# AmourWaltz/BayesLMs

Hardware: AMD Instinct MI355X
Metric: train_tokens_per_sec (higher is better)
Workload: dtype f32

## Files before the change

### bayeslms_amd/_lib.py

```python
import ctypes as C
import os

import torch

_HERE = os.path.dirname(os.path.abspath(__file__))
LIB_PATH = os.environ.get("BLM_LIB") or os.path.join(_HERE, "libbayeslm_hip.so")

ABI_VERSION = 1
TOPK_MAX = 256
OK = 0
ERR_INVALID, ERR_ABI, ERR_HIP, ERR_UNSUPPORTED = -1, -2, -3, -4
GEMM_NT, GEMM_NN, GEMM_TN = 0, 1, 2
EPI_NONE, EPI_BIAS, EPI_BIAS_GELU, EPI_MUL_DGELU, EPI_BAYES_WGRAD, EPI_GP_MIX, EPI_MUL_DGP_MIX = range(7)
GEMM_ACCUMULATE = 1
STREAM_WEIGHT = 0x10000000
STREAM_DROPOUT = 0x20000000
STREAM_LRT = 0x30000000

c_fp = C.POINTER(C.c_float)
c_i64p = C.POINTER(C.c_int64)


class Rng(C.Structure):
    _fields_ = [("seed", C.c_uint64), ("stream", C.c_uint32), ("step", C.c_uint32)]
# ... 32 lines not shown


class BeamPoolArgs(C.Structure):
    _fields_ = ([("abi_version", C.c_uint32), ("P", C.c_int32)]
                + [(n, C.c_void_p) for n in ("norm", "raw", "len", "step", "parent", "finished", "count", "inserted")])


class GemmPlan(C.Structure):
    _fields_ = [("tile", C.c_int32), ("splits", C.c_int32), ("source", C.c_int32), ("model_us", C.c_float)]


_vp, _i, _f, _i64 = C.c_void_p, C.c_int, C.c_float, C.c_int64
_rngp, _varp = C.POINTER(Rng), C.POINTER(Variational)
SIGNATURES = {
    "blm_abi_version": (C.c_uint32, []),
    "blm_last_error": (C.c_char_p, []),
    "blm_query": (_i, [_i, C.c_char_p, C.POINTER(_i), C.POINTER(_i)]),
    "blm_sample_weight": (_i, [_vp, _i64, _i64, _varp, _vp, _vp, _f, _vp]),
    "blm_sample_weight_bwd": (_i, [_vp, _i64, _i64, _varp, _vp, _vp, _vp]),
    "blm_variational_group_fwd": (_i, [C.POINTER(VarItem), _i, _vp, _vp]),
    "blm_variational_group_bwd": (_i, [C.POINTER(VarItem), _i, _vp, _vp]),
    "blm_philox_normal": (_i, [_vp, _i64, _rngp, _vp]),
    "blm_lrt_prepare": (_i, [_vp, _vp, _i64, _i, _vp]),
    "blm_lrt_combine": (_i, [_vp, _vp, _vp, _rngp, _i, _i, _i, _i, _i, _vp]),
    "blm_lrt_bwd_factor": (_i, [_vp, _vp, _vp, _vp, _rngp, _i, _i, _i, _i, _i, _vp]),
    "blm_lrt_mul": (_i, [_vp, _vp, _vp, _i64, _f, _i, _vp]),
    "blm_kl_mean_fwd": (_i, [_vp, _i64, _vp, _i64, _i64, _i, _f, _vp, _vp]),
    "blm_kl_mean_bwd": (_i, [_vp, _i64, _vp, _i64, _i64, _vp, _f, _vp, _i64, _vp, _vp]),
    "blm_gemm": (_i, [C.POINTER(GemmArgs), _vp]),
    "blm_set_gemm_mode": (_i, [_i]),
    "blm_get_gemm_mode": (_i, []),
    "blm_gemm_plan_query": (_i, [C.POINTER(GemmArgs), C.POINTER(GemmPlan)]),
    "blm_gemm_plan_launch": (_i, [C.POINTER(GemmArgs), C.POINTER(GemmPlan)]),
    "blm_gemm_plan_model_us": (_i, [C.POINTER(GemmArgs), _i, _i, C.POINTER(C.c_float)]),
    "blm_gemm_plan_override": (_i, [_i, _i]),
    "blm_gemm_plan_set": (_i, [_i] * 8),
    "blm_gemm_plan_clear": (_i, [_i]),
    "blm_mfma_probe_ws_floats": (_i64, []),
    "blm_mfma_probe": (_i, [_vp, _i, C.POINTER(C.c_double), _vp]),
    "blm_set_option": (_i, [C.c_char_p, _i]),
    "blm_get_option": (_i, [C.c_char_p, C.POINTER(C.c_int)]),
    "blm_gemm_plan_set_cus": (_i, [_i]),
    "blm_gemm_plan_get_cus": (_i, []),
    "blm_gemm_plan_comm_window": (_i, [_f]),
    "blm_gemm_plan_comm_window_left": (_f, []),
    "blm_gemm_plan_set_comm": (_i, [_i, _i, _i, _i, _i, _i, _i, _i]),
    "blm_embed_fwd": (_i, [_vp, _vp, _vp, _vp, _i, _i, _i, _i64, _f, _f, _rngp, _i, _i, _vp]),
    "blm_embed_bwd": (_i, [_vp, _vp, _vp, _i, _i, _i, _i64, _f, _f, _rngp, _i, _i, _vp]),
    "blm_add_pe_dropout": (_i, [_vp, _vp, _vp, _i, _i, _i, _f, _rngp, _i, _i, _vp]),
    "blm_dropout": (_i, [_vp, _vp, _i, _i, _i, _f, _rngp, _i, _i, _vp]),
    "blm_dropout_rows": (_i, [_vp, _vp, _i, _i, _i, _i, _f, _rngp, _i, _i, _vp]),
    "blm_add_dropout_ln_fwd": (_i, [_vp, _vp, _vp, _vp, _vp, _vp, _vp, _vp, _i, _i, _i, _f, _f, _rngp, _i, _i, _vp]),
    "blm_ln_bwd_ws_floats": (_i64, [_i, _i]),
    "blm_add_dropout_ln_bwd": (_i, [_vp, _vp, _vp, _vp, _vp, _vp, _vp, _vp, _vp, _vp, _i, _i, _i, _f, _rngp, _i, _i, _vp]),
    "blm_attn_fwd": (_i, [_vp, _vp, _vp, _i64, _vp, _vp, _i, _i, _i, _i, _f, _rngp, _i, _i, _vp]),
    "blm_attn_fwd_rows": (_i, [_vp, _vp, _vp, _i64, _vp, _vp, _i, _i, _i, _i, _vp]),
    "blm_attn_fwd_tree": (_i, [_vp, _vp, _vp, _i64, _vp, _vp, _vp, _i, _i, _i, _vp]),
    "blm_attn_bwd": (_i, [_vp, _vp, _vp, _i64, _vp, _vp, _vp, _vp, _vp, _vp, _i64, _i, _i, _i, _i, _f, _rngp, _i, _i, _vp]),
    "blm_attn_bwd_ws": (_i, [_vp, _vp, _vp, _i64, _vp, _vp, _vp, _vp, _vp, _vp, _i64, _i, _i, _i, _i, _f, _rngp, _i, _i, _vp,
                            _i64, _vp]),
    "blm_attn_bwd_ws_floats": (_i64, [_i, _i, _i, _i]),
    "blm_attn_fwd_keep": (_i, [_vp, _vp, _vp, _i64, _vp, _vp, _i, _i, _i, _i, _vp, _i, _i, _vp]),
    "blm_attn_bwd_keep": (_i, [_vp, _vp, _vp, _i64, _vp, _vp, _vp, _vp, _vp, _vp, _i64, _i, _i, _i, _i, _vp, _i, _i, _vp]),
    "blm_attn_decode_ws_floats": (_i64, [_i, _i, _i, _i, _i]),
    "blm_attn_decode": (_i, [_vp, _i64, _vp, _vp, _vp, _vp, _vp, _i64, _i, _i, _i, _i, _i, _i, _i, _vp]),
    "blm_kv_append": (_i, [_vp, _vp, _i64, _vp, _vp, _vp, _i, _i, _i, _i, _i, _i, _vp]),
    "blm_kv_gather": (_i, [_vp, _vp, _vp, _vp, _vp, _i, _i, _i, _i, _i, _i, _i, _vp]),
    "blm_embed_at": (_i, [_vp, _vp, _i64, _f, _vp, _vp, _i, _vp, _vp, _i, _i, _i, _vp]),
    "blm_log_softmax_rows": (_i, [_vp, _i64, _vp, _i64, _i, _i, _vp]),
    "blm_sample_rows": (_i, [_vp, _i64, _i, _i, _f, _rngp, _vp, _vp]),
    "blm_row_stats": (_i, [_vp, _i64, _vp, _i, _i, _vp, _vp, _vp, _vp, _vp, _vp]),
    "blm_topk_rows": (_i, [_vp, _i64, _i, _i, _i, _vp, _vp, _vp]),
    "blm_beam_select": (_i, [_vp, _vp, _vp, _vp, _i, _i, _i, _i64, _vp, _vp, _vp, _vp, _vp]),
    "blm_beam_select_pool": (_i, [_vp, _vp, _vp, _vp, _i, _i, _i, _i, _i64, _i, _i, _i, _f, _f, _i, C.POINTER(BeamPoolArgs),
                                  _vp, _vp, _vp, _vp, _vp, _vp, _vp]),
    "blm_sample_rows_filtered": (_i, [_vp, _i64, _i, _i, _f, _i, _f, _rngp, _vp, _vp]),
    "blm_ce_fwd_bwd": (_i, [_vp, _i64, _vp, _vp, _vp, _vp, _vp, _f, _i, _i, _vp]),
    "blm_ce_interp_fwd": (_i, [_vp, _vp, _i64, _f, _vp, _vp, _i, _i, _vp]),
    "blm_ce_soft_fwd_bwd": (_i, [_vp, _i64, _vp, _i64, _vp, _f, _vp, _vp, _vp, _vp, _vp, _vp, _vp, _f, _i, _i, _vp]),
    "blm_linear_nll_ws_floats": (_i64, [_i, _i]),
    "blm_linear_nll": (_i, [_vp, _i64, _vp, _i64, _vp, _vp, _vp, _vp, _vp, _i, _i, _i, _vp]),
    "blm_linear_mc_stats_ws_floats": (_i64, [_i, _i, _i]),
    "blm_linear_mc_stats": (_i, [_vp, _i64, _vp, _i64, _vp, _vp, _i, _vp, _vp, _vp, _vp, _vp, _i, _i, _i, _vp]),
    "blm_linear_mc_logprobs_ws_floats": (_i64, [_i, _i, _i]),
    "blm_linear_mc_logprobs": (_i, [_vp, _i64, _vp, _i64, _vp, _vp, _i, _vp, _i64, _vp, _vp, _vp, _vp, _vp, _i, _i, _i, _vp]),
    "blm_linear_nll2_wcat_floats": (_i64, [_i, _i, _i]),
    "blm_linear_nll2_ws_floats": (_i64, [_i, _i, _i, _i]),
    "blm_linear_nll2": (_i, [_vp, _i64, _vp, _i64, _vp, _i, _vp, _i64, _vp, _i64, _vp, _i, _f, _vp, _vp, _vp, _vp, _i, _vp, _i, _i, _vp]),
    "blm_linear_nll_edges_ws_floats": (_i64, [_i, _i]),
    "blm_linear_nll_edges": (_i, [_vp, _i64, _vp, _i64, _vp, _vp, _vp, _vp, _vp, _i, _i, _i, _i, _i, _vp]),
    "blm_linear_nll2_edges_ws_floats": (_i64, [_i, _i, _i, _i]),
    "blm_linear_nll2_edges": (_i, [_vp, _i64, _vp, _i64, _vp, _i, _vp, _i64, _vp, _i64, _vp, _i, _f, _vp, _vp, _vp, _vp, _i, _vp, _i, _i, _i,
                                   _vp]),
    "blm_ce_bwd": (_i, [_vp, _i64, _vp, _vp, _vp, _f, _vp, _i, _i, _vp]),
    "blm_gp_coef_grad": (_i, [_vp, _vp, _vp, _i, _i, _vp]),
    "blm_colsum": (_i, [_vp, _i64, _vp, _i, _i, _i, _vp]),
    "blm_colsum2": (_i, [_vp, _i64, _vp, _vp, _i, _i, _i, _vp]),
    "blm_init_multi": (_i, [_i, _vp, _vp, _vp, _vp, _vp]),
    "blm_sqnorm_ws_floats": (_i64, [_i]),
    "blm_sqnorm_multi": (_i, [_vp, _vp, _i, _vp, _vp, _vp]),
    "blm_clip_sgd_multi": (_i, [_vp, _vp, _vp, _vp, _i, _vp, _f, _f, _f, _i, _f, _vp]),
    "blm_lstm_step_fwd": (_i, [_vp, _vp, _vp, _vp, _vp, _vp, _vp, _vp, _i, _i, _vp]),
    "blm_lstm_step_bwd": (_i, [_vp] * 10 + [_i, _i, _vp]),
    "blm_lstm_seq_fwd": (_i, [_vp] * 6 + [_i, _i, _i, _vp]),
    "blm_lstm_seq_bwd": (_i, [_vp] * 7 + [_i, _vp, _i, _i, _i, _i, _i, _vp]),
    "blm_lstm_seq_pair_fwd": (_i, [_vp] * 5 + [_i] + [_vp] * 5 + [_i, _i, _i, _vp]),
# ... 172 lines not shown
```

### bayeslms_amd/csrc/elementwise.hip

```cpp
#include "blm_device.h"
#include "blm_host.h"
#include "blm_dropkey.h"

namespace blm {

constexpr int TPB = 256;

__global__ __launch_bounds__(TPB) void embed_fwd_kernel(const int64_t* __restrict__ ids, const float* __restrict__ enc,
                                                        const float* __restrict__ pe, float* __restrict__ out, int T,
                                                        int B, int D, long vocab, float scale, DropKey dk, bool vec) {
  const int lane = threadIdx.x & 63;
  const long row = (long)blockIdx.x * (TPB / 64) + (threadIdx.x >> 6);
  if (row >= (long)T * B) return;
  const int t = (int)(row / B), b = (int)(row % B);
  long id = ids[row];
  if (id < 0 || id >= vocab) id = 0;
  const float* e = enc + id * D;
  const float* pp = pe ? pe + (long)t * D : nullptr;
  float* o = out + row * D;
  if (vec) {
    for (int j = lane * 4; j < D; j += 256) {
      float4 v = *reinterpret_cast<const float4*>(e + j);
      float4 q = pp ? *reinterpret_cast<const float4*>(pp + j) : make_float4(0.f, 0.f, 0.f, 0.f);
      const float4 kp = keep4(dk, t, b, j);
// ... 140 lines not shown
    const float dx = s[v].x - mean, dy = s[v].y - mean, dz = s[v].z - mean, dw = s[v].w - mean;
    var += dx * dx + dy * dy + dz * dz + dw * dw;
  }
  const float rstd = rsqrtf(wave_sum(var) / D + eps);
  if (lane == 0) {
    if (mean_o) mean_o[row] = mean;
    if (rstd_o) rstd_o[row] = rstd;
  }
#pragma unroll
  for (int v = 0; v < VPT; ++v) {
    const int j = (v * 64 + lane) * 4;
    if (RAG && j >= D) continue;
    const float4 g = *reinterpret_cast<const float4*>(gamma + j);
    const float4 be = *reinterpret_cast<const float4*>(beta + j);
    if (s_out) *reinterpret_cast<float4*>(s_out + row * D + j) = s[v];
    float4 o;
    o.x = (s[v].x - mean) * rstd * g.x + be.x; o.y = (s[v].y - mean) * rstd * g.y + be.y;
    o.z = (s[v].z - mean) * rstd * g.z + be.z; o.w = (s[v].w - mean) * rstd * g.w + be.w;
    *reinterpret_cast<float4*>(out + row * D + j) = o;
  }
}

__global__ __launch_bounds__(TPB) void add_drop_ln_fwd_generic(const float* __restrict__ x, const float* __restrict__ y,
                                                               const float* __restrict__ gamma,
                                                               const float* __restrict__ beta, float* __restrict__ out,
                                                               float* __restrict__ s_buf, float* __restrict__ mean_o,
                                                               float* __restrict__ rstd_o, long M, float eps,
                                                               DropKey dk) {
  const int lane = threadIdx.x & 63, D = dk.D;
  const long row = (long)blockIdx.x * (TPB / 64) + (threadIdx.x >> 6);
  if (row >= M) return;
  const int t = (int)(row / dk.B), b = (int)(row % dk.B);
  float* s = s_buf + row * D;
  float sum = 0.f;
  for (int j = lane; j < D; j += 64) {
    const float v = x[row * D + j] + y[row * D + j] * keep1(dk, t, b, j);
    s[j] = v;
    sum += v;
  }
  const float mean = wave_sum(sum) / D;
  float var = 0.f;
  for (int j = lane; j < D; j += 64) {
    const float d = s[j] - mean;
    var += d * d;
  }
  const float rstd = rsqrtf(wave_sum(var) / D + eps);
  if (lane == 0) {
    if (mean_o) mean_o[row] = mean;
    if (rstd_o) rstd_o[row] = rstd;
  }
  for (int j = lane; j < D; j += 64) out[row * D + j] = (s[j] - mean) * rstd * gamma[j] + beta[j];
}

constexpr int LN_BWD_BLOCKS = 256;

template <int VPT, bool RAG = false>
__global__ __launch_bounds__(TPB) void add_drop_ln_bwd_reg(const float* __restrict__ dout, const float* __restrict__ s,
                                                           const float* __restrict__ gamma,
                                                           const float* __restrict__ mean_i,
                                                           const float* __restrict__ rstd_i, float* __restrict__ dx,
                                                           float* __restrict__ dy, float* __restrict__ ws, long M,
                                                           DropKey dk) {
  extern __shared__ __attribute__((aligned(16))) float sm[];
  const int lane = threadIdx.x & 63, wave = threadIdx.x >> 6, D = dk.D;
  float4 pg[VPT], pb[VPT], g[VPT];
#pragma unroll
  for (int v = 0; v < VPT; ++v) {
    pg[v] = pb[v] = make_float4(0.f, 0.f, 0.f, 0.f);
    g[v] = (RAG && (v * 64 + lane) * 4 >= D) ? make_float4(0.f, 0.f, 0.f, 0.f) : *reinterpret_cast<const float4*>(gamma + (v * 64 + lane) * 4);
  }
  for (long row = (long)blockIdx.x * 4 + wave; row < M; row += (long)gridDim.x * 4) {
    const int t = (int)(row / dk.B), b = (int)(row % dk.B);
    const float mean = mean_i[row], rstd = rstd_i[row];
    float4 xh[VPT], dxh[VPT];
    float s1 = 0.f, s2 = 0.f;
#pragma unroll
    for (int v = 0; v < VPT; ++v) {
      const int j = (v * 64 + lane) * 4;
      if (RAG && j >= D) { xh[v] = dxh[v] = make_float4(0.f, 0.f, 0.f, 0.f); continue; }
      const float4 d = *reinterpret_cast<const float4*>(dout + row * D + j);
      const float4 sv = *reinterpret_cast<const float4*>(s + row * D + j);
      xh[v] = make_float4((sv.x - mean) * rstd, (sv.y - mean) * rstd, (sv.z - mean) * rstd, (sv.w - mean) * rstd);
      dxh[v] = make_float4(d.x * g[v].x, d.y * g[v].y, d.z * g[v].z, d.w * g[v].w);
      pg[v].x += d.x * xh[v].x; pg[v].y += d.y * xh[v].y; pg[v].z += d.z * xh[v].z; pg[v].w += d.w * xh[v].w;
      pb[v].x += d.x; pb[v].y += d.y; pb[v].z += d.z; pb[v].w += d.w;
      s1 += dxh[v].x + dxh[v].y + dxh[v].z + dxh[v].w;
      s2 += dxh[v].x * xh[v].x + dxh[v].y * xh[v].y + dxh[v].z * xh[v].z + dxh[v].w * xh[v].w;
    }
    const float m1 = wave_sum(s1) / D, m2 = wave_sum(s2) / D;
#pragma unroll
    for (int v = 0; v < VPT; ++v) {
      const int j = (v * 64 + lane) * 4;
      if (RAG && j >= D) continue;
      float4 ds;
      ds.x = rstd * (dxh[v].x - m1 - xh[v].x * m2); ds.y = rstd * (dxh[v].y - m1 - xh[v].y * m2);
      ds.z = rstd * (dxh[v].z - m1 - xh[v].z * m2); ds.w = rstd * (dxh[v].w - m1 - xh[v].w * m2);
      *reinterpret_cast<float4*>(dx + row * D + j) = ds;
      if (dy) {
        const float4 kp = keep4(dk, t, b, j);
        ds.x *= kp.x; ds.y *= kp.y; ds.z *= kp.z; ds.w *= kp.w;
        *reinterpret_cast<float4*>(dy + row * D + j) = ds;
      }
    }
  }
#pragma unroll
  for (int v = 0; v < VPT; ++v) {
    const int j = (v * 64 + lane) * 4;
    if (RAG && j >= D) continue;
    *reinterpret_cast<float4*>(sm + (wave * 2 + 0) * D + j) = pg[v];
    *reinterpret_cast<float4*>(sm + (wave * 2 + 1) * D + j) = pb[v];
  }
  __syncthreads();
  for (int j = threadIdx.x; j < 2 * D; j += TPB) {
    const int which = j / D, c = j - which * D;
    ws[((long)blockIdx.x * 2 + which) * D + c] =
        sm[(0 * 2 + which) * D + c] + sm[(1 * 2 + which) * D + c] + sm[(2 * 2 + which) * D + c] + sm[(3 * 2 + which) * D + c];
  }
}

__global__ __launch_bounds__(TPB) void add_drop_ln_bwd_generic(const float* __restrict__ dout, const float* __restrict__ s,
                                                               const float* __restrict__ gamma,
                                                               const float* __restrict__ mean_i,
                                                               const float* __restrict__ rstd_i, float* __restrict__ dx,
                                                               float* __restrict__ dy, float* __restrict__ ws, long M,
                                                               DropKey dk) {
  const int lane = threadIdx.x & 63, wave = threadIdx.x >> 6, D = dk.D;
  float* wg = ws + (((long)blockIdx.x * 4 + wave) * 2 + 0) * D;
  float* wb = ws + (((long)blockIdx.x * 4 + wave) * 2 + 1) * D;
  for (long row = (long)blockIdx.x * 4 + wave; row < M; row += (long)gridDim.x * 4) {
    const int t = (int)(row / dk.B), b = (int)(row % dk.B);
    const float mean = mean_i[row], rstd = rstd_i[row];
    float s1 = 0.f, s2 = 0.f;
    for (int j = lane; j < D; j += 64) {
      const float d = dout[row * D + j], xh = (s[row * D + j] - mean) * rstd, dxh = d * gamma[j];
      s1 += dxh;
      s2 += dxh * xh;
      wg[j] += d * xh;
      wb[j] += d;
    }
    const float m1 = wave_sum(s1) / D, m2 = wave_sum(s2) / D;
    for (int j = lane; j < D; j += 64) {
      const float d = dout[row * D + j], xh = (s[row * D + j] - mean) * rstd;
      const float ds = rstd * (d * gamma[j] - m1 - xh * m2);
      dx[row * D + j] = ds;
      if (dy) dy[row * D + j] = ds * keep1(dk, t, b, j);
    }
  }
}

__global__ __launch_bounds__(TPB) void ln_bwd_finish(const float* __restrict__ ws, int nblk, int D,
                                                     float* __restrict__ dgamma, float* __restrict__ dbeta) {
  __shared__ float sm[2][4][64];
  const int c = threadIdx.x & 63, grp = threadIdx.x >> 6;
  const int j = blockIdx.x * 64 + c;
  float a = 0.f, b = 0.f;
  if (j < D) {
    int k = grp;
    for (; k + 28 < nblk; k += 32) {
      float ta[8], tb[8];
#pragma unroll
      for (int u = 0; u < 8; ++u) {
        ta[u] = ws[((long)(k + 4 * u) * 2 + 0) * D + j];
        tb[u] = ws[((long)(k + 4 * u) * 2 + 1) * D + j];
      }
#pragma unroll
      for (int u = 0; u < 8; ++u) { a += ta[u]; b += tb[u]; }
    }
    for (; k < nblk; k += 4) {
      a += ws[((long)k * 2 + 0) * D + j];
      b += ws[((long)k * 2 + 1) * D + j];
    }
  }
  sm[0][grp][c] = a;
  sm[1][grp][c] = b;
  __syncthreads();
  if (grp == 0 && j < D) {
    dgamma[j] += sm[0][0][c] + sm[0][1][c] + sm[0][2][c] + sm[0][3][c];
    dbeta[j] += sm[1][0][c] + sm[1][1][c] + sm[1][2][c] + sm[1][3][c];
  }
}

__global__ __launch_bounds__(TPB) void ce_kernel(const float* __restrict__ logits, long ld, const int64_t* __restrict__ tgt,
                                                 float* __restrict__ nll, float* __restrict__ lse_out,
                                                 float* __restrict__ dlogits, float gscale, int V) {
  __shared__ float red[TPB / 64];
  const long row = blockIdx.x;
  const float* x = logits + row * ld;
  float m = -INFINITY, l = 0.f;
  const bool vec = ((ld & 3) == 0) && ((reinterpret_cast<uintptr_t>(logits) & 15) == 0);
  const int V4 = vec ? (V & ~3) : 0;
  for (int j = threadIdx.x * 4; j < V4; j += TPB * 4) {
    const float4 v = *reinterpret_cast<const float4*>(x + j);
    const float mx = fmaxf(fmaxf(v.x, v.y), fmaxf(v.z, v.w));
    if (mx > m) { l *= __expf(m - mx); m = mx; }
    l += __expf(v.x - m) + __expf(v.y - m) + __expf(v.z - m) + __expf(v.w - m);
  }
  for (int j = V4 + threadIdx.x; j < V; j += TPB) {
    const float v = x[j];
    if (v > m) { l *= __expf(m - v); m = v; }
    l += __expf(v - m);
  }
  const long t = tgt[row];
  const bool valid = t >= 0 && t < V;
  const float xt = valid ? x[t] : 0.f;
  const float M_ = block_max<TPB / 64>(m, red);
  const float L_ = block_sum<TPB / 64>(m == -INFINITY ? 0.f : l * __expf(m - M_), red);
  const float lse = M_ + __logf(L_);
  if (threadIdx.x == 0) {
    nll[row] = valid ? lse - xt : 0.f;
    if (lse_out) lse_out[row] = lse;
  }
  if (dlogits) {
    if (!valid) gscale = 0.f;
    float* d = dlogits + row * ld;
    for (int j = threadIdx.x * 4; j < V4; j += TPB * 4) {
      float4 v = *reinterpret_cast<const float4*>(x + j);
      v.x = __expf(v.x - lse) * gscale; v.y = __expf(v.y - lse) * gscale;
      v.z = __expf(v.z - lse) * gscale; v.w = __expf(v.w - lse) * gscale;
      if (valid && t >= j && t < j + 4) {
        if (t == j) v.x -= gscale; else if (t == j + 1) v.y -= gscale; else if (t == j + 2) v.z -= gscale; else v.w -= gscale;
      }
      *reinterpret_cast<float4*>(d + j) = v;
    }
    for (int j = V4 + threadIdx.x; j < V; j += TPB) d[j] = (__expf(x[j] - lse) - ((valid && j == t) ? 1.f : 0.f)) * gscale;
  }
}

template <int NV>
__global__ __launch_bounds__(1024) void ce_row_kernel(const float* __restrict__ logits, long ld, const int64_t* __restrict__ tgt,
                                                      float* __restrict__ nll, float* __restrict__ lse_out,
                                                      float* __restrict__ dlogits, float gscale, int V) {
// ... 459 lines not shown
  DropKey dk = make_key(p, rng, B, D, col_offset, global_cols);
  dk.row0 = row0;
  const bool vec = D % 4 == 0 && ((reinterpret_cast<uintptr_t>(x) | reinterpret_cast<uintptr_t>(y)) & 15) == 0;
  hipLaunchKernelGGL(dropout_kernel, dim3(grid_for(n / 4 + 1)), dim3(TPB), 0, ST, x, y, (long)rows, dk, vec);
  BLM_HIP(hipGetLastError());
  return BLM_OK;
}

extern "C" int blm_add_pe_dropout(const float* x, const float* pe, float* out, int T, int B, int D, float p,
                                  const blm_rng* rng, int col_offset, int global_cols, void* stream) {
  if (!x || !pe || !out || !blm::extents_ok({T, B, D})) return blm_fail(BLM_ERR_INVALID, "blm_add_pe_dropout: bad arguments");
  if (p > 0.f && !rng) return blm_fail(BLM_ERR_INVALID, "blm_add_pe_dropout: dropout needs rng");
  const long n = (long)T * B * D;
  if (n == 0) return BLM_OK;
  hipLaunchKernelGGL(add_pe_dropout_kernel, dim3(grid_for(n)), dim3(TPB), 0, ST, x, pe, out, (long)T,
                     make_key(p, rng, B, D, col_offset, global_cols));
  BLM_HIP(hipGetLastError());
  return BLM_OK;
}

extern "C" int blm_add_dropout_ln_fwd(const float* x, const float* y, const float* gamma, const float* beta, float* out,
                                      float* s_out, float* mean, float* rstd, int rows, int B, int D, float eps_ln,
                                      float p, const blm_rng* rng, int col_offset, int global_cols, void* stream) {
  if (!x || !y || !gamma || !beta || !out || rows < 0 || B < 0 || D <= 0) return blm_fail(BLM_ERR_INVALID, "blm_add_dropout_ln_fwd: bad arguments");
  if (p > 0.f && !rng) return blm_fail(BLM_ERR_INVALID, "blm_add_dropout_ln_fwd: dropout needs rng");
  const long M = (long)rows * B;
  if (M == 0) return BLM_OK;
  const DropKey dk = make_key(p, rng, B, D, col_offset, global_cols);
  const dim3 grid((unsigned)((M + 3) / 4));
  const bool al = (((reinterpret_cast<uintptr_t>(x) | reinterpret_cast<uintptr_t>(y) | reinterpret_cast<uintptr_t>(out) |
                     reinterpret_cast<uintptr_t>(gamma) | reinterpret_cast<uintptr_t>(beta) | reinterpret_cast<uintptr_t>(s_out)) & 15) == 0);
#define LN_FWD(V) hipLaunchKernelGGL(add_drop_ln_fwd_reg<V>, grid, dim3(TPB), 0, ST, x, y, gamma, beta, out, s_out, mean, rstd, M, eps_ln, dk)
  if (al && D == 256) LN_FWD(1);
  else if (al && D == 512) LN_FWD(2);
  else if (al && D == 768) LN_FWD(3);
  else if (al && D == 1024) LN_FWD(4);
  else if (al && D == 1280) LN_FWD(5);
  else if (al && D == 1536) LN_FWD(6);
  else if (al && D == 2048) LN_FWD(8);
#define LN_FWD_RAG(V) hipLaunchKernelGGL((add_drop_ln_fwd_reg<V, true>), grid, dim3(TPB), 0, ST, x, y, gamma, beta, out, s_out, mean, rstd, M, eps_ln, dk)
  else if (al && D % 4 == 0 && D < 256) LN_FWD_RAG(1);
  else if (al && D % 4 == 0 && D < 512) LN_FWD_RAG(2);
  else if (al && D % 4 == 0 && D < 768) LN_FWD_RAG(3);
  else if (al && D % 4 == 0 && D < 1024) LN_FWD_RAG(4);
#undef LN_FWD_RAG
  else
    hipLaunchKernelGGL(add_drop_ln_fwd_generic, grid, dim3(TPB), 0, ST, x, y, gamma, beta, out, s_out ? s_out : out, mean,
                       rstd, M, eps_ln, dk);
#undef LN_FWD
  BLM_HIP(hipGetLastError());
  return BLM_OK;
}

extern "C" int64_t blm_ln_bwd_ws_floats(int M, int D) {
  (void)M;
  return (int64_t)2 * LN_BWD_BLOCKS * D;
}

extern "C" int blm_add_dropout_ln_bwd(const float* dout, const float* s, const float* gamma, const float* mean,
                                      const float* rstd, float* dx, float* dy, float* dgamma, float* dbeta, float* ws,
                                      int rows, int B, int D, float p, const blm_rng* rng, int col_offset,
                                      int global_cols, void* stream) {
  if (!dout || !s || !gamma || !mean || !rstd || !dx || !dgamma || !dbeta || !ws || rows < 0 || B < 0 || D <= 0)
    return blm_fail(BLM_ERR_INVALID, "blm_add_dropout_ln_bwd: bad arguments");
  if (p > 0.f && !rng) return blm_fail(BLM_ERR_INVALID, "blm_add_dropout_ln_bwd: dropout needs rng");
  const long M = (long)rows * B;
  if (M == 0) return BLM_OK;
  const DropKey dk = make_key(p, rng, B, D, col_offset, global_cols);
  int nblk = (int)((M + 3) / 4);
  if (nblk > LN_BWD_BLOCKS) nblk = LN_BWD_BLOCKS;
  const bool al = (((reinterpret_cast<uintptr_t>(dout) | reinterpret_cast<uintptr_t>(s) | reinterpret_cast<uintptr_t>(dx) |
                     reinterpret_cast<uintptr_t>(gamma) | reinterpret_cast<uintptr_t>(dy)) & 15) == 0);
  const size_t lds = (size_t)8 * D * sizeof(float);
#define LN_BWD(V) hipLaunchKernelGGL(add_drop_ln_bwd_reg<V>, dim3(nblk), dim3(TPB), lds, ST, dout, s, gamma, mean, rstd, dx, dy, ws, M, dk)
  if (al && D == 256) LN_BWD(1);
  else if (al && D == 512) LN_BWD(2);
  else if (al && D == 768) LN_BWD(3);
  else if (al && D == 1024) LN_BWD(4);
  else if (al && D == 1280) LN_BWD(5);
  else if (al && D == 1536) LN_BWD(6);
  else if (al && D == 2048) LN_BWD(8);
#define LN_BWD_RAG(V) hipLaunchKernelGGL((add_drop_ln_bwd_reg<V, true>), dim3(nblk), dim3(TPB), lds, ST, dout, s, gamma, mean, rstd, dx, dy, ws, M, dk)
  else if (al && D % 4 == 0 && D < 256) LN_BWD_RAG(1);
  else if (al && D % 4 == 0 && D < 512) LN_BWD_RAG(2);
  else if (al && D % 4 == 0 && D < 768) LN_BWD_RAG(3);
  else if (al && D % 4 == 0 && D < 1024) LN_BWD_RAG(4);
#undef LN_BWD_RAG
  else {
    nblk = (nblk + 3) / 4;
    BLM_HIP(hipMemsetAsync(ws, 0, (size_t)2 * 4 * nblk * D * sizeof(float), ST));
    hipLaunchKernelGGL(add_drop_ln_bwd_generic, dim3(nblk), dim3(TPB), 0, ST, dout, s, gamma, mean, rstd, dx, dy, ws, M, dk);
    nblk *= 4;
  }
#undef LN_BWD
  BLM_HIP(hipGetLastError());
  hipLaunchKernelGGL(ln_bwd_finish, dim3((D + 63) / 64), dim3(TPB), 0, ST, ws, nblk, D, dgamma, dbeta);
  BLM_HIP(hipGetLastError());
  return BLM_OK;
}

extern "C" int blm_ce_bwd(const float* logits, int64_t ld, const int64_t* tgt, const float* lse, const float* g_dev,
                          float scale, float* dlogits, int M, int V, void* stream) {
  if (!logits || !tgt || !lse || !g_dev || !dlogits || M < 0 || V <= 0 || ld < V) return blm_fail(BLM_ERR_INVALID, "blm_ce_bwd: bad arguments");
  if (M == 0) return BLM_OK;
  hipLaunchKernelGGL(ce_bwd_kernel, dim3(M), dim3(TPB), 0, ST, logits, (long)ld, tgt, lse, g_dev, scale, dlogits, V);
  BLM_HIP(hipGetLastError());
  return BLM_OK;
}

extern "C" int blm_ce_fwd_bwd(const float* logits, int64_t ld, const int64_t* tgt, float* nll, float* lse, float* loss_sum,
                              float* dlogits, float grad_scale, int M, int V, void* stream) {
  if (!logits || !tgt || !nll || M < 0 || V <= 0 || ld < V) return blm_fail(BLM_ERR_INVALID, "blm_ce_fwd_bwd: bad arguments");
  if (M == 0) return BLM_OK;
  const bool vec = ((ld & 3) == 0) && ((reinterpret_cast<uintptr_t>(logits) & 15) == 0) && (!dlogits || (reinterpret_cast<uintptr_t>(dlogits) & 15) == 0);
  if (vec && V <= 4096 * 3)
    hipLaunchKernelGGL(ce_row_kernel<3>, dim3(M), dim3(1024), 0, ST, logits, (long)ld, tgt, nll, lse, dlogits, grad_scale, V);
  else if (vec && V <= 4096 * 9)
    hipLaunchKernelGGL(ce_row_kernel<9>, dim3(M), dim3(1024), 0, ST, logits, (long)ld, tgt, nll, lse, dlogits, grad_scale, V);
  else if (vec && V <= 4096 * 16)
    hipLaunchKernelGGL(ce_row_kernel<16>, dim3(M), dim3(1024), 0, ST, logits, (long)ld, tgt, nll, lse, dlogits, grad_scale, V);
  else
    hipLaunchKernelGGL(ce_kernel, dim3(M), dim3(TPB), 0, ST, logits, (long)ld, tgt, nll, lse, dlogits, grad_scale, V);
  BLM_HIP(hipGetLastError());
  if (loss_sum) {
    hipLaunchKernelGGL(sum_kernel, dim3(1), dim3(1024), 0, ST, nll, (long)M, loss_sum);
    BLM_HIP(hipGetLastError());
  }
  return BLM_OK;
}

extern "C" int blm_ce_interp_fwd(const float* logits_a, const float* logits_b, int64_t ld, float alpha, const int64_t* tgt,
                                 float* nll, int M, int V, void* stream) {
  if (!logits_a || !logits_b || !tgt || !nll || M < 0 || V <= 0 || ld < V) return blm_fail(BLM_ERR_INVALID, "blm_ce_interp_fwd: bad arguments");
  if (M == 0) return BLM_OK;
  hipLaunchKernelGGL(ce_interp_kernel, dim3(M), dim3(TPB), 0, ST, logits_a, logits_b, (long)ld, alpha, tgt, nll, V);
  BLM_HIP(hipGetLastError());
  return BLM_OK;
}

extern "C" int blm_gp_coef_grad(const float* g, const float* z, float* dcoef, int M, int N, void* stream) {
  if (!g || !z || !dcoef || !blm::extents_ok({M, N})) return blm_fail(BLM_ERR_INVALID, "blm_gp_coef_grad: bad arguments");
  if (M == 0 || N == 0) return BLM_OK;
  int gy = (M + 127) / 128;
  if (gy > 64) gy = 64;
  if (blm::option(blm::OPT_DETERMINISTIC)) gy = 1;
  hipLaunchKernelGGL(gp_coef_grad_kernel, dim3((N + 63) / 64, gy), dim3(TPB), 0, ST, g, z, dcoef, M, N);
  BLM_HIP(hipGetLastError());
  return BLM_OK;
}
// ... 250 lines not shown
```

### include/bayeslm.h

```cpp
#ifndef BAYESLM_H
#define BAYESLM_H

#include <stdint.h>

#ifdef __cplusplus
extern "C" {
#endif

#define BLM_ABI_VERSION 1u

typedef enum blm_status {
  BLM_OK = 0,
  BLM_ERR_INVALID = -1,
  BLM_ERR_ABI = -2,
  BLM_ERR_HIP = -3,
  BLM_ERR_UNSUPPORTED = -4
} blm_status;

#define BLM_STREAM_WEIGHT  0x10000000u
#define BLM_STREAM_DROPOUT 0x20000000u
#define BLM_STREAM_LRT     0x30000000u

typedef struct blm_rng {
  uint64_t seed;
// ... 120 lines not shown
                    const int64_t* tgt, float* nll, float* lse, float* wcat, int pack_w, float* ws, int M, int N, void* stream);

int64_t blm_linear_nll_edges_ws_floats(int M, int N);
int blm_linear_nll_edges(const float* x, int64_t ldx, const float* w, int64_t ldw, const float* bias, const int64_t* edge_node,
                         const int64_t* edge_tgt, float* nll, float* ws, int M, int E, int N, int nv, int K, void* stream);
int64_t blm_linear_nll2_edges_ws_floats(int M, int N, int K1, int K2);
int blm_linear_nll2_edges(const float* x1, int64_t ldx1, const float* w1, int64_t ldw1, const float* b1, int K1,
                          const float* x2, int64_t ldx2, const float* w2, int64_t ldw2, const float* b2, int K2, float alpha,
                          const int64_t* edge_node, const int64_t* edge_tgt, float* nll, float* wcat, int pack_w, float* ws, int M, int E,
                          int N, void* stream);

int64_t blm_mfma_probe_ws_floats(void);
int blm_mfma_probe(float* ws, int iters, double* flops, void* stream);
int blm_set_option(const char* name, int value);
int blm_get_option(const char* name, int* value);

typedef struct blm_gemm_plan {
  int32_t tile;
  int32_t splits;
  int32_t source;
  float model_us;
} blm_gemm_plan;
int blm_gemm_plan_query(const blm_gemm_args* a, blm_gemm_plan* out);
int blm_gemm_plan_launch(const blm_gemm_args* a, blm_gemm_plan* out);
int blm_gemm_plan_model_us(const blm_gemm_args* a, int tile, int splits, float* us);
int blm_gemm_plan_override(int tile, int splits);
int blm_gemm_plan_set(int op, int M, int N, int K, int epilogue, int accumulate, int tile, int splits);
int blm_gemm_plan_clear(int keep_builtin);
int blm_gemm_plan_set_cus(int cus);
int blm_gemm_plan_get_cus(void);
int blm_gemm_plan_comm_window(float us);
float blm_gemm_plan_comm_window_left(void);
int blm_gemm_plan_set_comm(int op, int M, int N, int K, int epilogue, int accumulate, int tile, int splits);


int blm_embed_fwd(const int64_t* ids, const float* enc, const float* pe, float* out, int T, int B, int D,
                  int64_t vocab, float scale, float p, const blm_rng* rng, int col_offset, int global_cols,
                  void* stream);
int blm_embed_bwd(const int64_t* ids, const float* dy, float* denc, int T, int B, int D, int64_t vocab, float scale,
                  float p, const blm_rng* rng, int col_offset, int global_cols, void* stream);

int blm_add_pe_dropout(const float* x, const float* pe, float* out, int T, int B, int D, float p, const blm_rng* rng,
                       int col_offset, int global_cols, void* stream);

int blm_dropout(const float* x, float* y, int rows, int B, int D, float p, const blm_rng* rng, int col_offset,
                int global_cols, void* stream);
int blm_dropout_rows(const float* x, float* y, int rows, int row0, int B, int D, float p, const blm_rng* rng, int col_offset,
                     int global_cols, void* stream);

int blm_add_dropout_ln_fwd(const float* x, const float* y, const float* gamma, const float* beta, float* out,
                           float* s_out, float* mean, float* rstd, int rows, int B, int D, float eps_ln, float p,
                           const blm_rng* rng, int col_offset, int global_cols, void* stream);
int64_t blm_ln_bwd_ws_floats(int M, int D);
int blm_add_dropout_ln_bwd(const float* dout, const float* s, const float* gamma, const float* mean, const float* rstd,
                           float* dx, float* dy, float* dgamma, float* dbeta, float* ws, int rows, int B, int D,
                           float p, const blm_rng* rng, int col_offset, int global_cols, void* stream);

int blm_attn_fwd(const float* q, const float* k, const float* v, int64_t ld_qkv, float* out, float* lse, int T, int B,
                 int nhead, int head_dim, float p, const blm_rng* rng, int col_offset, int global_cols, void* stream);
int blm_attn_bwd(const float* q, const float* k, const float* v, int64_t ld_qkv, const float* out, const float* dout,
                 const float* lse, float* dq, float* dk, float* dv, int64_t ld_dqkv, int T, int B, int nhead,
                 int head_dim, float p, const blm_rng* rng, int col_offset, int global_cols, void* stream);
int blm_attn_fwd_rows(const float* q, const float* k, const float* v, int64_t ld_qkv, float* out, const int32_t* rowmap, int T,
                      int B, int nhead, int head_dim, void* stream);
int blm_attn_fwd_tree(const float* q, const float* k, const float* v, int64_t ld_qkv, float* out, const int32_t* end, const int32_t* lo,
                      int R, int nhead, int head_dim, void* stream);
int64_t blm_attn_bwd_ws_floats(int T, int B, int nhead, int head_dim);
int blm_attn_bwd_ws(const float* q, const float* k, const float* v, int64_t ld_qkv, const float* out, const float* dout,
                    const float* lse, float* dq, float* dk, float* dv, int64_t ld_dqkv, int T, int B, int nhead,
                    int head_dim, float p, const blm_rng* rng, int col_offset, int global_cols, float* ws,
                    int64_t ws_floats, void* stream);
int blm_attn_fwd_keep(const float* q, const float* k, const float* v, int64_t ld_qkv, float* out, float* lse, int T, int B, int nhead,
                      int head_dim, const float* keep, int col_offset, int global_cols, void* stream);
int blm_attn_bwd_keep(const float* q, const float* k, const float* v, int64_t ld_qkv, const float* out, const float* dout,
                      const float* lse, float* dq, float* dk, float* dv, int64_t ld_dqkv, int T, int B, int nhead, int head_dim,
                      const float* keep, int col_offset, int global_cols, void* stream);


int64_t blm_attn_decode_ws_floats(int Tq, int N, int nhead, int ctx_max, int head_dim);
int blm_attn_decode(const float* q, int64_t ld_q, const float* kv, const int32_t* past, const int32_t* n_new, float* out, float* ws,
                    int64_t ws_floats, int Tq, int N, int n_cap, int nhead, int max_len, int head_dim, int ctx_max, void* stream);
int blm_kv_append(const float* k, const float* v, int64_t ld_kv, float* kv, const int32_t* past, const int32_t* n_new, int Tq, int N,
                  int n_cap, int nhead, int max_len, int head_dim, void* stream);
int blm_kv_gather(const float* src, float* dst, const int64_t* idx, const int32_t* len, int32_t* len_out, int M, int n_src, int n_cap,
                  int outer, int nhead, int max_len, int head_dim, void* stream);
int blm_embed_at(const int64_t* ids, const float* enc, int64_t vocab, float scale, const float* x, const float* pe, int pe_rows,
                 const int32_t* pos0, float* out, int Tq, int N, int D, void* stream);
int blm_log_softmax_rows(const float* x, int64_t ldx, float* out, int64_t ldo, int R, int V, void* stream);
int blm_sample_rows(const float* x, int64_t ldx, int R, int V, float temperature, const blm_rng* rng, int64_t* out, void* stream);
int blm_row_stats(const float* x, int64_t ldx, const int64_t* tgt, int R, int V, float* nll, float* conf, float* entropy,
                  int32_t* pred, int32_t* rank, void* stream);

#define BLM_TOPK_MAX 256
int blm_topk_rows(const float* x, int64_t ldx, int R, int V, int k, float* vals, int64_t* ids, void* stream);
int blm_beam_select(const float* cand_vals, const int64_t* cand_ids, const float* score, const uint8_t* finished, int G, int B, int k,
                    int64_t eos, float* score_out, uint8_t* finished_out, int64_t* parent, int64_t* token, void* stream);
typedef struct blm_beam_pool {
  uint32_t abi_version;
  int32_t P;
  float* norm;
  float* raw;
  int32_t* len;
  int32_t* step;
  int64_t* parent;
  uint8_t* finished;
  int32_t* count;
// ... 145 lines not shown
```

Before: 410,400.

## Restructure LayerNorm backward: multi-row waves, wider blocks, vectorized partial reduction

The fused add-dropout-LayerNorm backward kernel now processes several rows per wave for small D, using 8-wave blocks and up to 512 partial-sum blocks. All loads for a row group are issued before any compute so more memory requests are in flight. The block-level dgamma/dbeta partial write happens only on the final iteration, and the finish kernel reads the partials with float4 loads and reduces them with wave shuffles. Workspace sizing changes to match the new part count, which raises register pressure and workspace size in exchange for better memory-level parallelism.

```diff
diff --git a/bayeslms_amd/_lib.py b/bayeslms_amd/_lib.py
--- a/bayeslms_amd/_lib.py
+++ b/bayeslms_amd/_lib.py
@@ -108,6 +108,7 @@
     "blm_dropout_rows": (_i, [_vp, _vp, _i, _i, _i, _i, _f, _rngp, _i, _i, _vp]),
     "blm_add_dropout_ln_fwd": (_i, [_vp, _vp, _vp, _vp, _vp, _vp, _vp, _vp, _i, _i, _i, _f, _f, _rngp, _i, _i, _vp]),
     "blm_ln_bwd_ws_floats": (_i64, [_i, _i]),
+    "blm_ln_bwd_partial_rows": (_i, [_i, _i, C.POINTER(C.c_int)]),
     "blm_add_dropout_ln_bwd": (_i, [_vp, _vp, _vp, _vp, _vp, _vp, _vp, _vp, _vp, _vp, _i, _i, _i, _f, _rngp, _i, _i, _vp]),
     "blm_attn_fwd": (_i, [_vp, _vp, _vp, _i64, _vp, _vp, _i, _i, _i, _i, _f, _rngp, _i, _i, _vp]),
     "blm_attn_fwd_rows": (_i, [_vp, _vp, _vp, _i64, _vp, _vp, _i, _i, _i, _i, _vp]),
diff --git a/bayeslms_amd/csrc/elementwise.hip b/bayeslms_amd/csrc/elementwise.hip
--- a/bayeslms_amd/csrc/elementwise.hip
+++ b/bayeslms_amd/csrc/elementwise.hip
@@ -216,69 +216,104 @@
   for (int j = lane; j < D; j += 64) out[row * D + j] = (s[j] - mean) * rstd * gamma[j] + beta[j];
 }
 
-constexpr int LN_BWD_BLOCKS = 256;
-
-template <int VPT, bool RAG = false>
-__global__ __launch_bounds__(TPB) void add_drop_ln_bwd_reg(const float* __restrict__ dout, const float* __restrict__ s,
-                                                           const float* __restrict__ gamma,
-                                                           const float* __restrict__ mean_i,
-                                                           const float* __restrict__ rstd_i, float* __restrict__ dx,
-                                                           float* __restrict__ dy, float* __restrict__ ws, long M,
-                                                           DropKey dk) {
+constexpr int LN_BWD_PARTS_GENERIC = 256;
+constexpr int ln_bwd_rows(int vpt) { return vpt <= 3 ? 2 : 1; }
+constexpr int ln_bwd_waves(int vpt) { return vpt <= 3 ? 8 : 4; }
+constexpr int ln_bwd_max_parts(int vpt) { return vpt <= 3 ? 512 : 256; }
+
+template <int VPT, bool RAG = false, int R = ln_bwd_rows(VPT), int NW = ln_bwd_waves(VPT)>
+__global__ __launch_bounds__(NW * 64) void add_drop_ln_bwd_reg(const float* __restrict__ dout, const float* __restrict__ s,
+                                                               const float* __restrict__ gamma,
+                                                               const float* __restrict__ mean_i,
+                                                               const float* __restrict__ rstd_i, float* __restrict__ dx,
+                                                               float* __restrict__ dy, float* __restrict__ ws, long M,
+                                                               DropKey dk) {
   extern __shared__ __attribute__((aligned(16))) float sm[];
-  const int lane = threadIdx.x & 63, wave = threadIdx.x >> 6, D = dk.D;
+  const int lane = threadIdx.x & 63, wave = __builtin_amdgcn_readfirstlane(threadIdx.x >> 6), D = dk.D;
+  const float4 zero = make_float4(0.f, 0.f, 0.f, 0.f);
+  const long stride = (long)gridDim.x * (NW * R);
   float4 pg[VPT], pb[VPT], g[VPT];
 #pragma unroll
   for (int v = 0; v < VPT; ++v) {
-    pg[v] = pb[v] = make_float4(0.f, 0.f, 0.f, 0.f);
-    g[v] = (RAG && (v * 64 + lane) * 4 >= D) ? make_float4(0.f, 0.f, 0.f, 0.f) : *reinterpret_cast<const float4*>(gamma + (v * 64 + lane) * 4);
-  }
-  for (long row = (long)blockIdx.x * 4 + wave; row < M; row += (long)gridDim.x * 4) {
-    const int t = (int)(row / dk.B), b = (int)(row % dk.B);
-    const float mean = mean_i[row], rstd = rstd_i[row];
-    float4 xh[VPT], dxh[VPT];
-    float s1 = 0.f, s2 = 0.f;
-#pragma unroll
-    for (int v = 0; v < VPT; ++v) {
-      const int j = (v * 64 + lane) * 4;
-      if (RAG && j >= D) { xh[v] = dxh[v] = make_float4(0.f, 0.f, 0.f, 0.f); continue; }
-      const float4 d = *reinterpret_cast<const float4*>(dout + row * D + j);
-      const float4 sv = *reinterpret_cast<const float4*>(s + row * D + j);
-      xh[v] = make_float4((sv.x - mean) * rstd, (sv.y - mean) * rstd, (sv.z - mean) * rstd, (sv.w - mean) * rstd);
-      dxh[v] = make_float4(d.x * g[v].x, d.y * g[v].y, d.z * g[v].z, d.w * g[v].w);
-      pg[v].x += d.x * xh[v].x; pg[v].y += d.y * xh[v].y; pg[v].z += d.z * xh[v].z; pg[v].w += d.w * xh[v].w;
-      pb[v].x += d.x; pb[v].y += d.y; pb[v].z += d.z; pb[v].w += d.w;
-      s1 += dxh[v].x + dxh[v].y + dxh[v].z + dxh[v].w;
-      s2 += dxh[v].x * xh[v].x + dxh[v].y * xh[v].y + dxh[v].z * xh[v].z + dxh[v].w * xh[v].w;
-    }
-    const float m1 = wave_sum(s1) / D, m2 = wave_sum(s2) / D;
-#pragma unroll
-    for (int v = 0; v < VPT; ++v) {
-      const int j = (v * 64 + lane) * 4;
-      if (RAG && j >= D) continue;
-      float4 ds;
-      ds.x = rstd * (dxh[v].x - m1 - xh[v].x * m2); ds.y = rstd * (dxh[v].y - m1 - xh[v].y * m2);
-      ds.z = rstd * (dxh[v].z - m1 - xh[v].z * m2); ds.w = rstd * (dxh[v].w - m1 - xh[v].w * m2);
-      *reinterpret_cast<float4*>(dx + row * D + j) = ds;
-      if (dy) {
-        const float4 kp = keep4(dk, t, b, j);
-        ds.x *= kp.x; ds.y *= kp.y; ds.z *= kp.z; ds.w *= kp.w;
-        *reinterpret_cast<float4*>(dy + row * D + j) = ds;
+    pg[v] = pb[v] = zero;
+    g[v] = (RAG && (v * 64 + lane) * 4 >= D) ? zero : *reinterpret_cast<const float4*>(gamma + (v * 64 + lane) * 4);
+  }
+  for (long base = (long)blockIdx.x * (NW * R); base < M; base += stride) {
+    const long row0 = base + (long)wave * R;
+    float4 xh[R][VPT], dxh[R][VPT];
+    float mean[R], rstd[R], s1[R], s2[R];
+#pragma unroll
+    for (int r = 0; r < R; ++r) {
+      const long row = row0 + r;
+      const bool live = row < M;
+      mean[r] = live ? mean_i[row] : 0.f;
+      rstd[r] = live ? rstd_i[row] : 0.f;
+#pragma unroll
+      for (int v = 0; v < VPT; ++v) {
+        const int j = (v * 64 + lane) * 4;
+        if (!live || (RAG && j >= D)) { xh[r][v] = dxh[r][v] = zero; continue; }
+        dxh[r][v] = *reinterpret_cast<const float4*>(dout + row * D + j);
+        xh[r][v] = *reinterpret_cast<const float4*>(s + row * D + j);
       }
     }
-  }
-#pragma unroll
-  for (int v = 0; v < VPT; ++v) {
-    const int j = (v * 64 + lane) * 4;
-    if (RAG && j >= D) continue;
-    *reinterpret_cast<float4*>(sm + (wave * 2 + 0) * D + j) = pg[v];
-    *reinterpret_cast<float4*>(sm + (wave * 2 + 1) * D + j) = pb[v];
-  }
-  __syncthreads();
-  for (int j = threadIdx.x; j < 2 * D; j += TPB) {
-    const int which = j / D, c = j - which * D;
-    ws[((long)blockIdx.x * 2 + which) * D + c] =
-        sm[(0 * 2 + which) * D + c] + sm[(1 * 2 + which) * D + c] + sm[(2 * 2 + which) * D + c] + sm[(3 * 2 + which) * D + c];
+#pragma unroll
+    for (int r = 0; r < R; ++r) {
+      s1[r] = s2[r] = 0.f;
+#pragma unroll
+      for (int v = 0; v < VPT; ++v) {
+        const float4 d = dxh[r][v], sv = xh[r][v];
+        const bool dead = row0 + r >= M || (RAG && (v * 64 + lane) * 4 >= D);
+        const float4 x = dead ? zero : make_float4((sv.x - mean[r]) * rstd[r], (sv.y - mean[r]) * rstd[r], (sv.z - mean[r]) * rstd[r], (sv.w - mean[r]) * rstd[r]);
+        const float4 e = make_float4(d.x * g[v].x, d.y * g[v].y, d.z * g[v].z, d.w * g[v].w);
+        xh[r][v] = x;
+        dxh[r][v] = e;
+        pg[v].x += d.x * x.x; pg[v].y += d.y * x.y; pg[v].z += d.z * x.z; pg[v].w += d.w * x.w;
+        pb[v].x += d.x; pb[v].y += d.y; pb[v].z += d.z; pb[v].w += d.w;
+        s1[r] += e.x + e.y + e.z + e.w;
+        s2[r] += e.x * x.x + e.y * x.y + e.z * x.z + e.w * x.w;
+      }
+    }
+    if (base + stride >= M) {
+#pragma unroll
+      for (int v = 0; v < VPT; ++v) {
+        const int j = (v * 64 + lane) * 4;
+        if (RAG && j >= D) continue;
+        *reinterpret_cast<float4*>(sm + (wave * 2 + 0) * D + j) = pg[v];
+        *reinterpret_cast<float4*>(sm + (wave * 2 + 1) * D + j) = pb[v];
+      }
+      __syncthreads();
+      for (int j = threadIdx.x; j < 2 * D; j += NW * 64) {
+        const int which = j / D, c = j - which * D;
+        float sum = sm[which * D + c];
+#pragma unroll
+        for (int w = 1; w < NW; ++w) sum += sm[(w * 2 + which) * D + c];
+        ws[((long)blockIdx.x * 2 + which) * D + c] = sum;
+      }
+    }
+#pragma unroll
+    for (int r = 0; r < R; ++r) { s1[r] = wave_sum(s1[r]) / D; s2[r] = wave_sum(s2[r]) / D; }
+#pragma unroll
+    for (int r = 0; r < R; ++r) {
+      const long row = row0 + r;
+      if (row >= M) continue;
+      const int t = (int)(row / dk.B), b = (int)(row % dk.B);
+      const float m1 = s1[r], m2 = s2[r];
+#pragma unroll
+      for (int v = 0; v < VPT; ++v) {
+        const int j = (v * 64 + lane) * 4;
+        if (RAG && j >= D) continue;
+        const float4 e = dxh[r][v], x = xh[r][v];
+        float4 ds;
+        ds.x = rstd[r] * (e.x - m1 - x.x * m2); ds.y = rstd[r] * (e.y - m1 - x.y * m2);
+        ds.z = rstd[r] * (e.z - m1 - x.z * m2); ds.w = rstd[r] * (e.w - m1 - x.w * m2);
+        *reinterpret_cast<float4*>(dx + row * D + j) = ds;
+        if (dy) {
+          const float4 kp = keep4(dk, t, b, j);
+          ds.x *= kp.x; ds.y *= kp.y; ds.z *= kp.z; ds.w *= kp.w;
+          *reinterpret_cast<float4*>(dy + row * D + j) = ds;
+        }
+      }
+    }
   }
 }
 
@@ -312,35 +347,47 @@
   }
 }
 
-__global__ __launch_bounds__(TPB) void ln_bwd_finish(const float* __restrict__ ws, int nblk, int D,
-                                                     float* __restrict__ dgamma, float* __restrict__ dbeta) {
-  __shared__ float sm[2][4][64];
-  const int c = threadIdx.x & 63, grp = threadIdx.x >> 6;
-  const int j = blockIdx.x * 64 + c;
-  float a = 0.f, b = 0.f;
-  if (j < D) {
-    int k = grp;
-    for (; k + 28 < nblk; k += 32) {
-      float ta[8], tb[8];
+template <int CW, int CG>
+__global__ __launch_bounds__(TPB) void ln_bwd_finish(const float* __restrict__ ws, int parts, int D, float* __restrict__ dgamma,
+                                                     float* __restrict__ dbeta) {
+  constexpr int RG = TPB / CG;
+  __shared__ float sm[4][CG][CW];
+  const int cg = threadIdx.x % CG, rg = threadIdx.x / CG, wave = threadIdx.x >> 6;
+  const int q = (blockIdx.x * CG + cg) * CW;
+  float acc[CW];
+#pragma unroll
+  for (int i = 0; i < CW; ++i) acc[i] = 0.f;
+  if (q < 2 * D) {
+    for (int k = rg; k < parts; k += 8 * RG) {
+      float t[8][CW];
 #pragma unroll
       for (int u = 0; u < 8; ++u) {
-        ta[u] = ws[((long)(k + 4 * u) * 2 + 0) * D + j];
-        tb[u] = ws[((long)(k + 4 * u) * 2 + 1) * D + j];
+        const int kk = k + u * RG;
+        if constexpr (CW == 4) {
+          const float4 v = kk < parts ? *reinterpret_cast<const float4*>(ws + (long)kk * 2 * D + q) : make_float4(0.f, 0.f, 0.f, 0.f);
+          t[u][0] = v.x; t[u][1] = v.y; t[u][2] = v.z; t[u][3] = v.w;
+        } else {
+          t[u][0] = kk < parts ? ws[(long)kk * 2 * D + q] : 0.f;
+        }
       }
 #pragma unroll
-      for (int u = 0; u < 8; ++u) { a += ta[u]; b += tb[u]; }
-    }
-    for (; k < nblk; k += 4) {
-      a += ws[((long)k * 2 + 0) * D + j];
-      b += ws[((long)k * 2 + 1) * D + j];
-    }
-  }
-  sm[0][grp][c] = a;
-  sm[1][grp][c] = b;
+      for (int u = 0; u < 8; ++u)
+#pragma unroll
+        for (int i = 0; i < CW; ++i) acc[i] += t[u][i];
+    }
+  }
+#pragma unroll
+  for (int o = 32; o >= CG; o >>= 1)
+#pragma unroll
+    for (int i = 0; i < CW; ++i) acc[i] += __shfl_xor(acc[i], o, 64);
+  if ((threadIdx.x & 63) < CG)
+#pragma unroll
+    for (int i = 0; i < CW; ++i) sm[wave][cg][i] = acc[i];
   __syncthreads();
-  if (grp == 0 && j < D) {
-    dgamma[j] += sm[0][0][c] + sm[0][1][c] + sm[0][2][c] + sm[0][3][c];
-    dbeta[j] += sm[1][0][c] + sm[1][1][c] + sm[1][2][c] + sm[1][3][c];
+  if (threadIdx.x < CG && q < 2 * D) {
+    float* out = q < D ? dgamma + q : dbeta + (q - D);
+#pragma unroll
+    for (int i = 0; i < CW; ++i) out[i] += sm[0][cg][i] + sm[1][cg][i] + sm[2][cg][i] + sm[3][cg][i];
   }
 }
 
@@ -906,9 +953,32 @@
   return BLM_OK;
 }
 
+static int ln_bwd_vpt(int D) {
+  if (D % 4 != 0 || D > 2048) return 0;
+  if (D <= 1024 || D == 1280 || D == 1536 || D == 2048) return (D + 255) / 256;
+  return 0;
+}
+static int ln_bwd_parts_reg(long M, int vpt) {
+  const long per = (long)ln_bwd_rows(vpt) * ln_bwd_waves(vpt);
+  const long n = (M + per - 1) / per, cap = ln_bwd_max_parts(vpt);
+  return (int)(n < cap ? n : cap);
+}
+static int ln_bwd_parts_generic(long M) {
+  const long n = (M + 3) / 4;
+  return 4 * (int)(((n < LN_BWD_PARTS_GENERIC ? n : LN_BWD_PARTS_GENERIC) + 3) / 4);
+}
+
+extern "C" int blm_ln_bwd_partial_rows(int M, int D, int* rows) {
+  if (!rows || M < 0 || D <= 0) return blm_fail(BLM_ERR_INVALID, "blm_ln_bwd_partial_rows: bad arguments");
+  const int vpt = ln_bwd_vpt(D), gen = ln_bwd_parts_generic(M > 0 ? M : 1), reg = vpt ? ln_bwd_parts_reg(M > 0 ? M : 1, vpt) : 0;
+  *rows = reg > gen ? reg : gen;
+  return BLM_OK;
+}
+
 extern "C" int64_t blm_ln_bwd_ws_floats(int M, int D) {
-  (void)M;
-  return (int64_t)2 * LN_BWD_BLOCKS * D;
+  int rows = 0;
+  if (M < 0 || D <= 0 || blm_ln_bwd_partial_rows(M, D, &rows) != BLM_OK) return 0;
+  return (int64_t)2 * rows * D;
 }
 
 extern "C" int blm_add_dropout_ln_bwd(const float* dout, const float* s, const float* gamma, const float* mean,
@@ -921,34 +991,38 @@
   const long M = (long)rows * B;
   if (M == 0) return BLM_OK;
   const DropKey dk = make_key(p, rng, B, D, col_offset, global_cols);
-  int nblk = (int)((M + 3) / 4);
-  if (nblk > LN_BWD_BLOCKS) nblk = LN_BWD_BLOCKS;
   const bool al = (((reinterpret_cast<uintptr_t>(dout) | reinterpret_cast<uintptr_t>(s) | reinterpret_cast<uintptr_t>(dx) |
                      reinterpret_cast<uintptr_t>(gamma) | reinterpret_cast<uintptr_t>(dy)) & 15) == 0);
-  const size_t lds = (size_t)8 * D * sizeof(float);
-#define LN_BWD(V) hipLaunchKernelGGL(add_drop_ln_bwd_reg<V>, dim3(nblk), dim3(TPB), lds, ST, dout, s, gamma, mean, rstd, dx, dy, ws, M, dk)
-  if (al && D == 256) LN_BWD(1);
-  else if (al && D == 512) LN_BWD(2);
-  else if (al && D == 768) LN_BWD(3);
-  else if (al && D == 1024) LN_BWD(4);
-  else if (al && D == 1280) LN_BWD(5);
-  else if (al && D == 1536) LN_BWD(6);
-  else if (al && D == 2048) LN_BWD(8);
-#define LN_BWD_RAG(V) hipLaunchKernelGGL((add_drop_ln_bwd_reg<V, true>), dim3(nblk), dim3(TPB), lds, ST, dout, s, gamma, mean, rstd, dx, dy, ws, M, dk)
-  else if (al && D % 4 == 0 && D < 256) LN_BWD_RAG(1);
-  else if (al && D % 4 == 0 && D < 512) LN_BWD_RAG(2);
-  else if (al && D % 4 == 0 && D < 768) LN_BWD_RAG(3);
-  else if (al && D % 4 == 0 && D < 1024) LN_BWD_RAG(4);
-#undef LN_BWD_RAG
-  else {
-    nblk = (nblk + 3) / 4;
-    BLM_HIP(hipMemsetAsync(ws, 0, (size_t)2 * 4 * nblk * D * sizeof(float), ST));
-    hipLaunchKernelGGL(add_drop_ln_bwd_generic, dim3(nblk), dim3(TPB), 0, ST, dout, s, gamma, mean, rstd, dx, dy, ws, M, dk);
-    nblk *= 4;
+  const int vpt = al ? ln_bwd_vpt(D) : 0;
+  int parts;
+#define LN_BWD_LAUNCH(V, RAG)                                                                                                     \
+  hipLaunchKernelGGL((add_drop_ln_bwd_reg<V, RAG>), dim3(parts), dim3(ln_bwd_waves(V) * 64),                                      \
+                     (size_t)ln_bwd_waves(V) * 2 * D * sizeof(float), ST, dout, s, gamma, mean, rstd, dx, dy,   \
+                     ws, M, dk)
+#define LN_BWD(V)                       \
+  case V:                               \
+    if (D == 256 * V) LN_BWD_LAUNCH(V, false); \
+    else LN_BWD_LAUNCH(V, true);        \
+    break
+  if (vpt) {
+    parts = ln_bwd_parts_reg(M, vpt);
+    switch (vpt) {
+      LN_BWD(1); LN_BWD(2); LN_BWD(3); LN_BWD(4);
+      case 5: LN_BWD_LAUNCH(5, false); break;
+      case 6: LN_BWD_LAUNCH(6, false); break;
+      default: LN_BWD_LAUNCH(8, false); break;
+    }
+  } else {
+    parts = ln_bwd_parts_generic(M);
+    BLM_HIP(hipMemsetAsync(ws, 0, (size_t)2 * parts * D * sizeof(float), ST));
+    hipLaunchKernelGGL(add_drop_ln_bwd_generic, dim3(parts / 4), dim3(TPB), 0, ST, dout, s, gamma, mean, rstd, dx, dy, ws, M, dk);
   }
 #undef LN_BWD
-  BLM_HIP(hipGetLastError());
-  hipLaunchKernelGGL(ln_bwd_finish, dim3((D + 63) / 64), dim3(TPB), 0, ST, ws, nblk, D, dgamma, dbeta);
+#undef LN_BWD_LAUNCH
+  BLM_HIP(hipGetLastError());
+  const bool vec = D % 4 == 0 && (((reinterpret_cast<uintptr_t>(ws) | reinterpret_cast<uintptr_t>(dgamma) | reinterpret_cast<uintptr_t>(dbeta)) & 15) == 0);
+  if (vec) hipLaunchKernelGGL((ln_bwd_finish<4, 8>), dim3((2 * D + 31) / 32), dim3(TPB), 0, ST, ws, parts, D, dgamma, dbeta);
+  else hipLaunchKernelGGL((ln_bwd_finish<1, 32>), dim3((2 * D + 31) / 32), dim3(TPB), 0, ST, ws, parts, D, dgamma, dbeta);
   BLM_HIP(hipGetLastError());
   return BLM_OK;
 }
diff --git a/include/bayeslm.h b/include/bayeslm.h
--- a/include/bayeslm.h
+++ b/include/bayeslm.h
@@ -196,6 +196,7 @@
                            float* s_out, float* mean, float* rstd, int rows, int B, int D, float eps_ln, float p,
                            const blm_rng* rng, int col_offset, int global_cols, void* stream);
 int64_t blm_ln_bwd_ws_floats(int M, int D);
+int blm_ln_bwd_partial_rows(int M, int D, int* rows);
 int blm_add_dropout_ln_bwd(const float* dout, const float* s, const float* gamma, const float* mean, const float* rstd,
                            float* dx, float* dy, float* dgamma, float* dbeta, float* ws, int rows, int B, int D,
                            float p, const blm_rng* rng, int col_offset, int global_cols, void* stream);
```

New measurement: 411,900 (median of 6 runs). No clear change (+0.4%).
